# OSU-NLP-Group/saev

Hardware: AMD Instinct MI355X
Metric: activations/sec (train step), d_in=1024 x32 k=32 (higher is better)
Workload: dtype f32 (encoder: fp16 MFMA first pass with a rigorous error margin, survivors recomputed exactly in fp32; all else fp32)

## Files before the change

### saev_amd/csrc/ctx.h

```cpp
#pragma once
#include <hip/hip_runtime.h>

#include <algorithm>
#include <cmath>
#include <cstdio>
#include <cstdlib>
#include <cstring>
#include <string>
#include <vector>

#include "kernels.h"

constexpr int AUX_KSPLIT_MAX = 16;
constexpr int CAND_CAP = 4096;
constexpr int CAND_STRIDE = CAND_CAP + 256;
constexpr int TIMING_RING = 512;
constexpr int DEAD_LAG = 4;
constexpr int DEAD_RING = 16;
enum { AUX_NONE = 0, AUX_SMALL_DEVICE = 1, AUX_SMALL_HOST = 2, AUX_DENSE = 3 };

struct saev_ctx {
    saev_cfg cfg{};
    saev_debug_cfg dbg{};
    int device = 0;
// ... 42 lines not shown
    float2* row_proj = nullptr;
    float* enc_sq = nullptr;
    bool row_proj_valid = false, tail_proj_in_adam = false;
    bool wenc_t_pending = false;
    int64_t* toks = nullptr;
    int32_t *fired = nullptr, *dead = nullptr;
    int32_t* flags = nullptr;
    int32_t *chunk_starts = nullptr, *part_starts = nullptr, *work_latent = nullptr;
    float *dW_encT = nullptr, *partials = nullptr, *db_partials = nullptr;
    bool dws_ok = false;
    int dws_rows = 0;
    bool dws_pairs = false;
    float *gS = nullptr, *xS = nullptr, *dvp = nullptr;
    float* xS_ov = nullptr;
    float* xS_bwd = nullptr;
    float* dval_rows = nullptr;
    bool dval_fwd = false;
    float* wn2 = nullptr;
    float* sq_wave = nullptr;
    int sq_wave_n = 0;
    bool wn2_fresh = false;
    bool dval_pairs_ready = false;
    bool fused_forward = false;
    bool fwd_slices = false;
    bool fwd_step = false;
    float* rs_part = nullptr;
    float* xS_c = nullptr;
    int2 *pv = nullptr, *pv2 = nullptr;
    int32_t *plat = nullptr, *cut_lat = nullptr, *cut_list = nullptr;
    int32_t* lat_unused = nullptr;
    bool fused_step = false;
    bool unused_valid = false;
    int P = 1;
    int32_t cuts[MAX_PREFIXES] = {0};
    float* G = nullptr;
    float* GS = nullptr;
    int P_cap = 0;
    int n_dead_host = 0, k_use_host = 0;
    int64_t tokens_seen = 0;
    bool tracker_dirty = false;
    int nd_cap = 0;
    DeadRecord* rec_host = nullptr;
    DeadRecord* rec_dev = nullptr;
    hipEvent_t dead_ev[DEAD_RING];
    bool dead_ev_created = false;
    int64_t dead_steps = 0;
// ... 196 lines not shown
```

### saev_amd/csrc/ctx_backward.hip

```cpp
#include "ctx.h"

extern "C" {


int saev_backward_begin(saev_ctx* c, void* stream) {
    if (!c) return SAEV_INVALID_ARG;
    REQUIRE(c, !c->relu_train, SAEV_UNSUPPORTED, "saev_backward_begin: a ReLU training context runs its dense backward in one piece (saev_step_backward)");
    REQUIRE(c, c->x_last && c->training_last, SAEV_INVALID_ARG, "saev_backward_begin: no training forward in flight");
    REQUIRE(c, c->grads, SAEV_NOT_BOUND, "gradient buffer not bound");
    hipStream_t s = (hipStream_t)stream;
    const int S = c->cfg.d_sae, D = c->cfg.d_model, K = c->cfg.top_k;
    const bool ov = c->ov_x != nullptr;
    const int n = ov ? c->ov_n : c->n_last;
    const int words = ((n + 31) / 32 + 7) / 8 * 8;
    c->row_proj_valid = false;
    CscArgs a{};
    a.idx = ov ? c->ov_idx : c->idx; a.code_stride = K; a.k = K; a.k_dev = nullptr; a.n_rows = n; a.S = S;
    a.bitmap = c->bitmap; a.words = words; a.grp_prefix = c->grp_prefix; a.scan_totals = c->scan_totals;
    a.counts = c->counts; a.starts = c->starts; a.pairs = c->pairs;
    a.chunk_starts = c->chunk_starts; a.part_starts = c->part_starts; a.work_latent = c->work_latent;
    const bool ov_slices = ov && c->dws_ok && c->P_last == 1 && n <= c->back_rows;
    c->dws_pairs = ov ? ov_slices : c->dws_rows == n;
    if (ov_slices) {
        c->xS_bwd = c->xS;
        if (!c->followers.empty()) {
            if (c->xS_ov == nullptr) {
                int rca = alloc(c, &c->xS_ov, (size_t)c->back_rows * D);
                if (rca != SAEV_OK) return rca;
            }
            c->xS_bwd = c->xS_ov;
        }
        HIPCHK(c, launch_slice_major_copy(c->ov_g, c->ov_x, n, D, c->gS, c->xS_bwd, s));
        c->dws_rows = 0;
    }
    c->csc_epoch = c->csc_epoch == 0x7fffffff ? 1 : c->csc_epoch + 1;
    a.epoch = c->dbg.csc_route == 2 ? 0 : c->csc_epoch;
    if (c->dws_pairs) {
        a.zero_word = c->cut_list;
        a.pv = c->pv; a.plat = c->plat; a.val = ov ? c->ov_val : c->val;
        a.P = c->P_last;
        for (int p = 0; p < c->P_last; ++p) a.cuts[p] = c->cuts_last[p];
        if (!ov && c->dval_fwd) { a.pv2 = c->pv2; a.dval = c->dval_rows; }
    }
    c->dval_pairs_ready = c->dws_pairs && a.pv2 != nullptr;
    if (c->fused_step && c->dws_pairs) { a.pairs = nullptr; a.chunk_starts = nullptr; a.part_starts = nullptr; a.work_latent = nullptr; }
    const float* gmat = ov ? c->ov_g : (c->P_last > 1 ? c->G : c->g);
    const bool prefilled = !ov && c->bitmap_prefill_words == words && c->bitmap_prefill_rows == n;
    HIPCHK(c, launch_csc_build(a, s, c->bitmap_clean && words <= c->bitmap_clean_words, gmat, D, (long)c->P_last * D,
                               c->colsum_partials, c->grads + c->off_b_dec, prefilled));
    c->bitmap_prefill_words = 0;
    c->last_backward_gathered = ov;
    c->bitmap_clean = false;
    c->bitmap_words_last = words;
    if (c->aux_route != AUX_NONE) {
        int rc = auxk_backward(c, s);
        if (rc != SAEV_OK) return rc;
    }
    return SAEV_OK;
}

int saev_backward_rows(saev_ctx* c, int32_t lat_lo, int32_t lat_hi, void* stream) {
    return saev_backward_rows_part(c, lat_lo, lat_hi, 0, stream);
}

int saev_backward_rows_part(saev_ctx* c, int32_t lat_lo, int32_t lat_hi, int32_t part, void* stream) {
    if (!c) return SAEV_INVALID_ARG;
    REQUIRE(c, !c->relu_train, SAEV_UNSUPPORTED, "saev_backward_rows: a ReLU training context runs its dense backward in one piece, over all latents (saev_step_backward)");
    REQUIRE(c, part >= 0 && part <= 2, SAEV_INVALID_ARG, "saev_backward_rows_part: part must be 0 (both), 1 (decoder) or 2 (encoder)");
    REQUIRE(c, c->x_last && c->training_last && c->grads, SAEV_INVALID_ARG, "saev_backward_rows: call saev_backward_begin first");
    const int S = c->cfg.d_sae, D = c->cfg.d_model, K = c->cfg.top_k;
    const bool ov = c->ov_x != nullptr;
    const int n = ov ? c->ov_n : c->n_last;
    REQUIRE(c, 0 <= lat_lo && lat_lo < lat_hi && lat_hi <= S, SAEV_INVALID_ARG, "saev_backward_rows: bad latent range");
    REQUIRE(c, !c->btk || (part == 0 && lat_lo == 0 && lat_hi == S), SAEV_UNSUPPORTED,
            "saev_backward_rows: a BatchTopK context runs the backward over all latents in one part");
    hipStream_t s = (hipStream_t)stream;
    DwRowsArgs a{};
    a.starts = c->starts; a.chunk_starts = c->chunk_starts; a.work_latent = c->work_latent;
    a.part_starts = c->part_starts; a.pairs = c->pairs; a.val = ov ? c->ov_val : c->val; a.W_dec = c->params + c->off_W_dec;
    a.g = ov ? c->ov_g : (c->P_last > 1 ? c->G : c->g);
    a.x = ov ? c->ov_x : c->x_last;
    a.D = D; a.S = S; a.k_dev = nullptr; a.accumulate = 0;
    a.P = c->P_last;
    for (int p = 0; p < c->P_last; ++p) a.cuts[p] = c->cuts_last[p];
    a.dW_dec = c->grads + c->off_W_dec; a.dW_encT = c->dW_encT; a.db_enc = c->grads + c->off_b_enc;
    a.partials = c->partials; a.db_partials = c->db_partials;
    a.lat_lo = lat_lo; a.lat_hi = lat_hi;
    a.part = part; a.dval = c->dval_pairs;
    const bool all_rows = part == 0 && lat_lo == 0 && lat_hi == S;
    const bool clears = part != 2 && lat_lo == 0 && lat_hi == S && c->bitmap_words_last > 0;
    if (clears) { a.clear_bitmap = c->bitmap; a.clear_words = c->bitmap_words_last; }
    a.row_proj = all_rows ? c->row_proj : nullptr; a.project = c->cfg.remove_parallel_grads ? 1 : 0;
    a.enc_sq = all_rows ? c->enc_sq : nullptr;
    const int max_work = (lat_hi - lat_lo) + (int)(((long)n * K + DW_CHUNK - 1) / DW_CHUNK);
    if (lat_lo == 0 && lat_hi == S && c->dws_pairs && (ov || c->dws_rows == n)) {
        DwSlicesArgs w{};
        w.starts = c->starts; w.pv = c->pv; w.pv2 = c->pv2; w.plat = c->plat; w.gS = c->P_last > 1 ? c->GS : c->gS; w.W_dec = a.W_dec; w.P = c->P_last;
        w.xS = ov ? c->xS_bwd : (c->fwd_step ? c->xS_c : c->xS);
        w.n_rows = n; w.D = D; w.S = S; w.pair_cap = (int)((long)c->back_rows * K);
        w.dvp = c->dvp; w.dW_dec = a.dW_dec; w.dW_encT = a.dW_encT; w.db_enc = a.db_enc;
        const size_t runs_cap = ((size_t)w.pair_cap + DWS_RUN - 1) / DWS_RUN;
        w.part_dec = c->partials; w.part_enc = c->partials + 2 * runs_cap * D;
        w.cut_lat = c->cut_lat; w.cut_list = c->cut_list;
        w.lat_unused = (all_rows && c->fused_step) ? c->lat_unused : nullptr;
        c->unused_valid = w.lat_unused != nullptr;
        w.row_proj = a.row_proj; w.project = a.project; w.enc_sq = a.enc_sq;
        w.clear_bitmap = a.clear_bitmap; w.clear_words = a.clear_words;
        w.have_dval = c->dval_pairs_ready ? 1 : 0;
        c->sq_wave_n = 0;
        if (c->dval_pairs_ready && c->wn2_fresh && part == 0) {
            w.wn2 = c->wn2;
            if (c->fused_step && all_rows && c->sq_wave != nullptr && c->dbg.fin_route != 2) {
                c->sq_wave_n = dw_slices_waves(D, (int)((long)n * K));
                w.sq_wave_dec = c->sq_wave; w.sq_wave_enc = c->sq_wave + c->sq_wave_n;
            }
        }
        HIPCHK(c, launch_dw_slices(w, (int)((long)n * K), part, s));
    } else {
// ... 13 lines not shown
    if (ov && c->aux_route != AUX_NONE && part != 2 && lat_lo == 0)
        HIPCHK(c, launch_colsum(c->db_aux, 1, D, c->colsum_partials, c->grads + c->off_b_dec, 1, nullptr, s));
    c->row_proj_valid = all_rows;
    if (clears) { c->bitmap_clean = true; c->bitmap_clean_words = c->bitmap_words_last; }
    return SAEV_OK;
}

float* saev_grad_w_enc_t(saev_ctx* c) { return c ? c->dW_encT : nullptr; }

int saev_bind_w_enc_t(saev_ctx* c, float* scratch) {
    if (!c || !scratch) return SAEV_INVALID_ARG;
    c->dW_encT = scratch;
    return SAEV_OK;
}

int saev_copy_step_state(saev_ctx* c, int32_t n_rows, float* g_out, int32_t* idx_out, float* val_out, void* stream) {
    if (!c) return SAEV_INVALID_ARG;
    REQUIRE(c, !c->btk, SAEV_UNSUPPORTED, "saev_copy_step_state: not for a BatchTopK context (no sparse-state exchange)");
    REQUIRE(c, !c->relu_train, SAEV_UNSUPPORTED, "saev_copy_step_state: not for a ReLU training context (its step state is dense: no sparse-state exchange)");
    REQUIRE(c, c->n_last > 0 && c->training_last && n_rows == c->n_last, SAEV_INVALID_ARG,
            "saev_copy_step_state: n_rows must be the row count of the training forward in flight");
    hipStream_t s = (hipStream_t)stream;
    const size_t nk = (size_t)n_rows * c->cfg.top_k, nd = (size_t)n_rows * c->cfg.d_model * (size_t)c->P_last;
    if (g_out) HIPCHK(c, hipMemcpyAsync(g_out, c->P_last > 1 ? c->G : c->g, nd * sizeof(float), hipMemcpyDeviceToDevice, s));
    if (idx_out) HIPCHK(c, hipMemcpyAsync(idx_out, c->idx, nk * sizeof(int32_t), hipMemcpyDeviceToDevice, s));
    if (val_out) HIPCHK(c, hipMemcpyAsync(val_out, c->val, nk * sizeof(float), hipMemcpyDeviceToDevice, s));
    return SAEV_OK;
}

int saev_backward_override(saev_ctx* c, const float* x_all, const float* g_all, const int32_t* idx_all, const float* val_all,
                           int32_t n_all) {
    if (!c) return SAEV_INVALID_ARG;
    if (x_all == nullptr) { c->ov_x = nullptr; c->ov_n = 0; return SAEV_OK; }
    REQUIRE(c, !c->btk, SAEV_UNSUPPORTED, "saev_backward_override: not for a BatchTopK context (a batch-wide top-k over ranks needs a distributed select)");
    REQUIRE(c, !c->relu_train, SAEV_UNSUPPORTED, "saev_backward_override: not for a ReLU training context (one GPU: the dense backward runs over its own rows)");
    REQUIRE(c, g_all && idx_all && val_all && n_all > 0, SAEV_INVALID_ARG, "saev_backward_override: NULL buffer");
    REQUIRE(c, n_all <= c->back_rows, SAEV_INVALID_ARG,
            "saev_backward_override: the gathered row count exceeds saev_cfg.max_backward_rows (set it to the GLOBAL batch)");
    REQUIRE(c, c->x_last && c->training_last, SAEV_INVALID_ARG, "saev_backward_override: no training forward in flight");
    REQUIRE(c, ((uintptr_t)x_all % 16) == 0 && ((uintptr_t)g_all % 16) == 0, SAEV_INVALID_ARG, "x_all / g_all must be 16-byte aligned");
    c->ov_x = x_all; c->ov_g = g_all; c->ov_idx = idx_all; c->ov_val = val_all; c->ov_n = n_all;
    return SAEV_OK;
}

int32_t saev_aux_compact_rows(const saev_ctx* c) {
    if (!c || c->aux_route == AUX_NONE) return 0;
// ... 53 lines not shown
```

### saev_amd/csrc/ctx_forward.hip

```cpp
#include "ctx.h"

extern "C" {


int saev_normalize_w_dec(saev_ctx* c, void* stream) {
    if (!c) return SAEV_INVALID_ARG;
    REQUIRE(c, c->params, SAEV_NOT_BOUND, "parameters not bound");
    if (!c->cfg.normalize_w_dec) return SAEV_OK;
    HIPCHK(c, launch_normalize_rows(c->params + c->off_W_dec, c->cfg.d_sae, c->cfg.d_model, (hipStream_t)stream));
    return SAEV_OK;
}

static bool bind_x_sources(saev_ctx* c, const float* x, int n, bool allow_borrow) {
    saev_ctx* l = c->leader;
    const bool borrow = allow_borrow && l != nullptr && l->xprep_x == x && l->xprep_n == n && l->xprep_serial != c->leader_serial_seen;
    saev_ctx* src = borrow ? l : c;
    c->upper_c = src->upper; c->mu_c = src->mu; c->xnorm_c = src->xnorm; c->xabs_c = src->xabs_part; c->xs_c = src->xs;
    c->borrow_streamed = borrow && l->fwd_streamed && l->mu_keep != nullptr;
    if (c->borrow_streamed) c->mu_c = l->mu_keep;
    c->fwd_step = c->fwd_slices && (src == c || src->fwd_slices);
    c->xS_c = c->fwd_step ? src->xS : nullptr;
    if (borrow) c->leader_serial_seen = l->xprep_serial;
    return borrow;
}
// ... 230 lines not shown
            } else
            HIPCHK(c, launch_pre_encode(c->cand_cnt, n, c->gmax, ng * c->gmax_stride, f16r_mode ? c->xnorm_c : nullptr, c->cfg.d_model,
                                        c->wnorm_scratch, (S_ + 255) / 256, f16r_mode ? scl(c) : nullptr, const_cast<int32_t*>(pre_flag),
                                        c->wmax_prev, c->row_margin, c->flags + 1, s));
            timing_begin(c, s);
            int rc = run_encoder(c, x, n, EPI_TOPK, nullptr, pre_flag, 0, s);
            if (rc != SAEV_OK) return rc;
            timing_end(c, s);
            rc = select_stage(need_dense, 0, need_dense, nullptr, c->flags + 1, pre_flag);
            if (rc != SAEV_OK) return rc;
        }
    } else {
        HIPCHK(c, launch_init_i32(need_dense, 1, 1, s));
        HIPCHK(c, hipMemsetAsync(c->flags + 2, 0, 2 * sizeof(int32_t), s));
        timing_begin(c, s);
        timing_end(c, s);
    }
    int rc = run_encoder(c, x, n, EPI_DENSE, c->h_dense, need_dense, 1, s);
    if (rc != SAEV_OK) return rc;
    SelectDenseArgs sd{};
    sd.h = c->h_dense; sd.n_rows = n; sd.S = c->cfg.d_sae; sd.k = K;
    sd.idx_out = idx_out; sd.val_out = val_out; sd.out_stride = K;
    sd.enable_flag = need_dense; sd.enable_when = 1;
    HIPCHK(c, launch_select_dense(sd, s));
    return SAEV_OK;
}

int saev_encode_topk(saev_ctx* c, const float* x, int32_t n, int32_t* idx_out, float* val_out, void* stream) {
    if (!c) return SAEV_INVALID_ARG;
    REQUIRE(c, c->cfg.activation == SAEV_ACT_TOPK, SAEV_UNSUPPORTED,
            "saev_encode_topk: a TopK context only (ReLU: saev_encode_relu, BatchTopK: saev_encode_batch_topk)");
    REQUIRE(c, c->params, SAEV_NOT_BOUND, "parameters not bound");
    REQUIRE(c, x && idx_out && val_out && n > 0 && n <= c->cfg.max_batch, SAEV_INVALID_ARG,
            "saev_encode_topk: bad arguments (n_rows must be in 1..max_batch)");
    hipStream_t s = (hipStream_t)stream;
    HIPCHK(c, hipMemsetAsync(c->flags, 0, sizeof(int32_t), s));
    bind_x_sources(c, x, n, false);
    c->xprep_x = nullptr;
    c->stream_step = false;
    c->follow_stream = false;
    return encode_topk_impl(c, x, n, idx_out, val_out, c->flags, s);
}

int saev_scatter_dense(saev_ctx* c, const int32_t* idx, const float* val, int32_t n, int32_t k, float* f_out,
                       void* stream) {
    if (!c) return SAEV_INVALID_ARG;
// ... 246 lines not shown
        c->prep_valid = true;
    }
    if (wdec_ev != nullptr) HIPCHK(c, hipStreamWaitEvent(s, wdec_ev, 0));
    if (training) {
        c->wn2_fresh = false;
        if (c->cfg.normalize_w_dec) {
            HIPCHK(c, launch_normalize_rows(c->params + c->off_W_dec, S, D, s, c->wn2));
            c->wn2_fresh = c->wn2 != nullptr;
        }
    }

    DecodeArgs a{};
    a.x = x; a.idx = c->idx; a.val = c->val; a.code_stride = K; a.k = K;
    a.W_dec = c->params + c->off_W_dec; a.b_dec = c->params + c->off_b_dec;
    a.n_rows = n; a.D = D; a.S = S; a.idx_limit = S;
    a.upper = c->upper_c;
    a.gscale = 2.0f / ((float)n * (float)D * (float)c->P);
    a.training = training ? 1 : 0;
    a.g = c->g; a.x_hat = c->x_hat; a.fired = c->fired; a.rowstats = c->rowstats;
    c->dws_rows = 0;
    c->dval_fwd = false;
    if (training && c->dws_ok && (c->P == 1 || c->GS != nullptr)) { a.gS = c->P == 1 ? c->gS : c->GS; a.xS = c->fwd_step ? nullptr : c->xS; c->dws_rows = n; }
    if (c->dws_rows == n && c->dval_rows != nullptr && (c->P == 1 || decode_matry_forms_dval(D, K))) { a.dval_out = c->dval_rows; c->dval_fwd = true; }
    c->bitmap_prefill_words = 0;
    if (training && c->dbg.csc_route == 0 && c->bitmap != nullptr && c->bitmap_clean && !c->last_backward_gathered) {
        const int words = ((n + 31) / 32 + 7) / 8 * 8;
        if (words <= c->bitmap_clean_words) {
            a.csc_bitmap = c->bitmap; a.csc_words = words;
            c->bitmap_prefill_words = words; c->bitmap_prefill_rows = n;
            c->bitmap_clean = false;
        }
    }
    if (c->P > 1) {
        MatryArgs m{};
        m.P = c->P;
        for (int p = 0; p < c->P; ++p) m.cuts[p] = c->cuts[p];
        m.G = c->G;
        m.g_rows_all = c->fused_forward ? 0 : 1;
        HIPCHK(c, launch_decode_matry(a, m, s));
    } else {
        HIPCHK(c, launch_decode(a, s));
    }
    c->P_last = c->P;
    for (int p = 0; p < c->P; ++p) c->cuts_last[p] = c->cuts[p];
    const bool lists = !btk && fused_supported(c->cfg) && !(c->cfg.bound_mode != 0 && c->cfg.encoder_mode != SAEV_ENCODER_F32 && f16_ngroups(c) == 32);
    c->stats_pending = false;
// ... 12 lines not shown
```

### saev_amd/csrc/kernels.h

```cpp
#pragma once
#include <hip/hip_runtime.h>
#include <stdint.h>

#include <string>

#include "../../include/saev_amd.h"

enum { EPI_DENSE = 0, EPI_TOPK = 1 };

struct EncodeArgs {
    const float* x;
    const float* W_enc;
    const float* b_enc;
    int n_rows, D, S;
    int s_splits;
    float* h_out;
    int ngroups;
    int32_t* gmax;
    int gmax_stride;
    int32_t* cand_cnt;
    float* cand_val;
    int32_t* cand_idx;
    int cand_cap;
    int cand_stride;
    const int32_t* enable_flag;
    int enable_when;
};

size_t encode_gemm_smem_bytes();
hipError_t launch_encode_gemm(const EncodeArgs& a, int epi, hipStream_t stream);
int encode_gemm_tile_rows();
int encode_gemm_tile_latents();

struct SelectDenseArgs {
    const float* h;
    int n_rows, S;
    int k;
    const int32_t* k_dev;
    const int32_t* mask;
    int32_t* idx_out;
    float* val_out;
    int out_stride;
    const int32_t* enable_flag;
    int enable_when;
};
hipError_t launch_select_dense(const SelectDenseArgs& a, hipStream_t stream);

struct SelectCandArgs {
    const int32_t* cand_cnt;
    const float* cand_val;
    const int32_t* cand_idx;
    int cand_cap, cand_stride, n_rows, k;
    int32_t* idx_out;
    float* val_out;
    int out_stride;
    const int32_t* enable_flag;
    int enable_when;
    const float* row_margin;
    const float* x;
    const float* W_encT;
    const float* b_enc;
    int D;
    int32_t* surv_idx;
    float* surv_val;
    int32_t* surv_cnt;
    int32_t* refine_overflow;
    const int32_t* tau_max;
// ... 93 lines not shown
    int n_rows, S;
    uint32_t* bitmap;
    int words;
    int32_t* grp_prefix;
    int32_t* counts;
    int32_t* scan_totals;
    int32_t* starts;
    int2* pairs;
    int32_t* chunk_starts;
    int32_t* part_starts;
    int32_t* work_latent;
    int2* pv;
    int32_t* plat;
    const float* val;
    int2* pv2;
    const float* dval;
    int P;
    int32_t cuts[16];
    int32_t* zero_word;
    int32_t epoch;
};
hipError_t launch_csc_build(const CscArgs& a, hipStream_t stream, bool bitmap_clean = false, const float* colsum_m = nullptr,
                            int colsum_D = 0, long colsum_row_stride = 0, float* colsum_partials = nullptr,
                            float* colsum_out = nullptr, bool prefilled = false);

constexpr int DW_CHUNK = 64;

struct DwRowsArgs {
    const int32_t* starts;
    const int32_t* chunk_starts;
    const int32_t* work_latent;
    const int32_t* part_starts;
    const int2* pairs;
    const float* val;
    const float* W_dec;
    const float* g;
    const float* x;
    int D, S;
    int P;
    int32_t cuts[MAX_PREFIXES];
    const int32_t* k_dev;
    int accumulate;
    float* dW_dec;
    float* dW_encT;
    float* db_enc;
    float* partials;
    float* db_partials;
// ... 446 lines not shown
```

### saev_amd/csrc/select.hip

```cpp
#include "common.h"
#include "kernels.h"

namespace {

constexpr int SD_THREADS = 256;

__device__ __forceinline__ int block_excl_scan_256(int v, int* lds_wave_tot, int& total) {
    const int lane = threadIdx.x & 63, w = threadIdx.x >> 6;
    int incl = v;
#pragma unroll
    for (int o = 1; o < 64; o <<= 1) {
        int n = __shfl_up(incl, o, 64);
        if (lane >= o) incl += n;
    }
    if (lane == 63) lds_wave_tot[w] = incl;
    __syncthreads();
    int base = 0, tot = 0;
#pragma unroll
    for (int i = 0; i < 4; ++i) {
        const int t = lds_wave_tot[i];
        if (i < w) base += t;
        tot += t;
    }
    total = tot;
    __syncthreads();
    return base + incl - v;
}

__global__ __launch_bounds__(SD_THREADS) void select_dense_kernel(SelectDenseArgs a) {
    if (a.enable_flag != nullptr && (*a.enable_flag != 0) != (a.enable_when != 0)) return;
    __shared__ int hist[256];
    __shared__ int sh_digit, sh_need;
    __shared__ int wave_tot[4];

    const int row = blockIdx.x;
    const int S = a.S;
    int k = a.k_dev ? min(*a.k_dev, a.k) : a.k;
    if (a.k_dev && k <= 0) return;
    const float* h = a.h + (size_t)row * S;
    const int tid = threadIdx.x;
    const int S4 = S >> 2;

    uint32_t prefix = 0, pmask = 0;
    int need = k;

    for (int pass = 0; pass < 4; ++pass) {
        const int shift = 24 - 8 * pass;
        hist[tid] = 0;
        __syncthreads();
        for (int q = tid; q < S4; q += SD_THREADS) {
            const f32x4 v = *reinterpret_cast<const f32x4*>(h + 4 * q);
            int4 mk = {1, 1, 1, 1};
            if (a.mask) mk = *reinterpret_cast<const int4*>(a.mask + 4 * q);
            const int m[4] = {mk.x, mk.y, mk.z, mk.w};
#pragma unroll
            for (int e = 0; e < 4; ++e) {
                const uint32_t key = f2ukey(v[e]);
                if (m[e] != 0 && (key & pmask) == prefix) atomicAdd(&hist[(key >> shift) & 255], 1);
            }
        }
        __syncthreads();
        if (tid < 64) {
            const int c0 = hist[4 * tid], c1 = hist[4 * tid + 1], c2 = hist[4 * tid + 2], c3 = hist[4 * tid + 3];
            const int c = c0 + c1 + c2 + c3;
// ... 47 lines not shown
        const int neq = feq[0] + feq[1] + feq[2] + feq[3];
        int tot;
        const int ex = block_excl_scan_256(ngt | (neq << 16), wave_tot, tot);
        int gt_before = base_gt + (ex & 0xFFFF);
        int eq_before = base_eq + (ex >> 16);
#pragma unroll
        for (int e = 0; e < 4; ++e) {
            if (flg[e]) {
                const int pos = gt_before + min(eq_before, need);
                oi[pos] = 4 * q + e;
                ov[pos] = v[e];
                ++gt_before;
            } else if (feq[e]) {
                if (eq_before < need) {
                    const int pos = gt_before + eq_before;
                    oi[pos] = 4 * q + e;
                    ov[pos] = v[e];
                }
                ++eq_before;
            }
        }
        base_gt += tot & 0xFFFF;
        base_eq += tot >> 16;
    }
}


__device__ __forceinline__ float wave_reduce_scatter8(float (&p)[8], int lane) {
    int bit = 32;
#pragma unroll
    for (int h = 4; h >= 1; h >>= 1, bit >>= 1) {
        const bool up = (lane & bit) != 0;
#pragma unroll
        for (int i = 0; i < h; ++i) {
            const float keep = up ? p[i + h] : p[i];
            const float send = up ? p[i] : p[i + h];
            p[i] = keep + __shfl_xor(send, bit, 64);
        }
    }
    float r = p[0];
    for (; bit >= 1; bit >>= 1) r += __shfl_xor(r, bit, 64);
    return r;
}

__device__ __forceinline__ void sort_by_idx_and_store(const SelectCandArgs& a, int row, int k, int32_t my_idx, float my_val,
                                                      int lane) {
// ... 724 lines not shown
    if (state[5] > 0.f) { state[5] -= 1.f; g = 1; }
    *gate = g;
}
__global__ void heur_update_kernel(float* state, const int32_t* bad, const float* cand_mean, int k, const int32_t* gate) {
    if (threadIdx.x != 0 || *gate != 0) return;
    float z = state[0];
    state[2] += 1.f;
    if (*bad != 0) {
        z -= 0.3f;
        state[1] += 1.f;
        state[4] += 1.f;
        if (state[4] >= 3.f) { state[4] = 0.f; state[5] = 256.f; z = 1.5f; }
    } else {
        state[4] = 0.f;
        if (*cand_mean > 3.f * (float)k) z += 0.002f;
    }
    state[0] = fminf(fmaxf(z, 0.5f), 3.5f);
}

}

hipError_t launch_select_dense(const SelectDenseArgs& a, hipStream_t stream) {
    if (a.n_rows <= 0) return hipSuccess;
    hipLaunchKernelGGL(select_dense_kernel, dim3(a.n_rows), dim3(SD_THREADS), 0, stream, a);
    return hipGetLastError();
}

hipError_t launch_select_cand(const SelectCandArgs& a, hipStream_t stream) {
    if (a.n_rows <= 0) return hipSuccess;
    if (a.cand_cap > 4096 || (a.sum_part != nullptr && a.cand_cap > REFINE_CAP)) return hipErrorInvalidValue;
    if (a.k > 32) hipLaunchKernelGGL(select_cand_kernel<true>, dim3((a.n_rows + 3) / 4), dim3(256), 0, stream, a);
    else hipLaunchKernelGGL(select_cand_kernel<false>, dim3((a.n_rows + 3) / 4), dim3(256), 0, stream, a);
    return hipGetLastError();
}

hipError_t launch_init_i32(int32_t* p, int32_t v, int n, hipStream_t stream) {
    if (n <= 0) return hipSuccess;
    hipLaunchKernelGGL(init_i32_kernel, dim3((n + 255) / 256), dim3(256), 0, stream, p, v, n);
    return hipGetLastError();
}

hipError_t launch_encoder_init(int32_t* cand_cnt, int n_rows, int32_t* gmax, int n_gmax, hipStream_t stream, int32_t* tau_max,
                               const int32_t* enable_flag, int enable_when) {
    const int n = n_rows > n_gmax ? n_rows : n_gmax;
    if (n <= 0) return hipSuccess;
    hipLaunchKernelGGL(encoder_init_kernel, dim3((n + 255) / 256), dim3(256), 0, stream, cand_cnt, n_rows, gmax, n_gmax, tau_max,
                       enable_flag, enable_when);
// ... 96 lines not shown
```

### saev_amd/csrc/sparse.hip

```cpp
#include "common.h"
#include "kernels.h"

namespace {

template <int NV>
__device__ __forceinline__ void gather_rows_accum(f32x4 (&acc)[NV], const float* __restrict__ W, int D, int D4,
                                                  const int32_t* idx_row, const float* val_row, int k, int limit,
                                                  int lane) {
    for (int j0 = 0; j0 < k; j0 += 64) {
        const int cnt = min(64, k - j0);
        int32_t my_i = -1;
        float my_v = 0.f;
        if (lane < cnt) { my_i = idx_row[j0 + lane]; my_v = val_row[j0 + lane]; }
#pragma unroll 4
        for (int jj = 0; jj < cnt; ++jj) {
            const int32_t i = __shfl(my_i, jj, 64);
            const float v = __shfl(my_v, jj, 64);
            if (i < 0 || i >= limit) continue;
            const f32x4* wr = reinterpret_cast<const f32x4*>(W + (size_t)i * D);
#pragma unroll
            for (int n = 0; n < NV; ++n) {
                const int q = lane + 64 * n;
                if (q < D4) {
                    const f32x4 w = wr[q];
// ... 69 lines not shown
        return;
    }
    const float u = a.upper ? fmaxf(*a.upper, 1e-12f) : 1.0f;
    float sse_scaled = 0.f;
    double sse64 = 0.0, sumsq64 = 0.0;
    f32x4 g[NV];
    const f32x4* xr = reinterpret_cast<const f32x4*>(a.x + (size_t)row * D);
#pragma unroll
    for (int n = 0; n < NV; ++n) {
        const int q = lane + 64 * n;
        g[n] = f32x4{0.f, 0.f, 0.f, 0.f};
        if (q < D4) {
            const f32x4 xv = xr[q];
            if (a.x_hat) reinterpret_cast<f32x4*>(a.x_hat + (size_t)row * D)[q] = acc[n];
#pragma unroll
            for (int e = 0; e < 4; ++e) {
                const float t = acc[n][e] / u - xv[e] / u;
                sse_scaled += t * t * u * u;
                g[n][e] = a.gscale * t * u;
                const float r = xv[e] - acc[n][e];
                sse64 += (double)r * (double)r;
                sumsq64 += (double)xv[e] * (double)xv[e];
            }
            if (a.training) reinterpret_cast<f32x4*>(a.g + (size_t)row * D)[q] = g[n];
            if (a.training && a.gS != nullptr) {
                const size_t o = ((size_t)(q >> 3) * a.n_rows + row) * 8 + (q & 7);
                reinterpret_cast<f32x4*>(a.gS)[o] = g[n];
                if (a.xS != nullptr) reinterpret_cast<f32x4*>(a.xS)[o] = xv;
            }
        }
    }
    float l0 = 0.f, l1 = 0.f;
    for (int j = lane; j < a.k; j += 64) {
        const int32_t i = idx_row[j];
        const float v = val_row[j];
        if (i >= 0 && v != 0.f) {
            l0 += 1.f;
            l1 += fabsf(v);
            if (a.training && a.fired) a.fired[i] = 1;
        }
        csc_mark(a, i, row);
    }
    if (a.rowstats) {
        sse_scaled = wave_sum(sse_scaled);
        l0 = wave_sum(l0);
        l1 = wave_sum(l1);
        sse64 = wave_sum_d(sse64);
// ... 42 lines not shown
#pragma unroll
        for (int j = 0; j < 32; ++j) {
            const int i = __builtin_amdgcn_readlane(my_i, 32 * h + j);
            const float v = __builtin_bit_cast(float, __builtin_amdgcn_readlane(__builtin_bit_cast(int, raw_v), 32 * h + j));
            if (i >= 0) acc += v * wv[j];
        }
        __builtin_amdgcn_sched_barrier(0);
    }
    if (a.x_hat) reinterpret_cast<f32x4*>(a.x_hat + (size_t)row * a.D)[q] = acc;
    const float u = a.upper ? fmaxf(*a.upper, 1e-12f) : 1.0f;
    float sse_scaled = 0.f;
    double sse64 = 0.0, sumsq64 = 0.0;
    f32x4 g;
#pragma unroll
    for (int e = 0; e < 4; ++e) {
        const float t = acc[e] / u - xv[e] / u;
        sse_scaled += t * t * u * u;
        g[e] = a.gscale * t * u;
        const float r = xv[e] - acc[e];
        sse64 += (double)r * (double)r;
        sumsq64 += (double)xv[e] * (double)xv[e];
    }
    if (a.training) {
        reinterpret_cast<f32x4*>(a.g + (size_t)row * a.D)[q] = g;
        if (a.gS != nullptr) {
            const size_t o = ((size_t)(q >> 3) * a.n_rows + row) * 8 + (q & 7);
            reinterpret_cast<f32x4*>(a.gS)[o] = g;
            if (a.xS != nullptr) reinterpret_cast<f32x4*>(a.xS)[o] = xv;
        }
    }
#pragma unroll
    for (int hh = 0; hh < KH; ++hh) {
        const int h = KH - 1 - hh;
        if (hh > 0) {
#pragma unroll
            for (int j = 0; j < 32; ++j) {
                const int i = __builtin_amdgcn_readlane(my_i, 32 * h + j);
                const i32x4_ t = __builtin_amdgcn_raw_buffer_load_b128(wres, voff, (uint32_t)max(i, 0) * (uint32_t)(D4 * 16), 0);
                wv[j] = f32x4{__int_as_float(t[0]), __int_as_float(t[1]), __int_as_float(t[2]), __int_as_float(t[3])};
            }
            __builtin_amdgcn_sched_barrier(0);
        }
        float pd[32];
#pragma unroll
        for (int j = 0; j < 32; ++j) pd[j] = (g[0] * wv[j][0] + g[1] * wv[j][1]) + (g[2] * wv[j][2] + g[3] * wv[j][3]);
        const float r = wave_reduce_scatter32(pd, lane);
        if ((lane & 1) == 0) sh_dv[w][32 * h + (lane >> 1)] = r;
// ... 1220 lines not shown
    if (k_dev && col_mult > 0 && (int)blockIdx.x * 64 >= *k_dev * col_mult) return;
    __shared__ float part[4][64];
    const int col = threadIdx.x & 63, slice = threadIdx.x >> 6;
    const int d = blockIdx.x * 64 + col;
    float s0 = 0.f, s1 = 0.f, s2 = 0.f, s3 = 0.f;
    if (d < D) {
        int b = slice;
        for (; b + 12 < n_blocks; b += 16) {
            s0 += partials[(size_t)b * D + d];
            s1 += partials[(size_t)(b + 4) * D + d];
            s2 += partials[(size_t)(b + 8) * D + d];
            s3 += partials[(size_t)(b + 12) * D + d];
        }
        for (; b < n_blocks; b += 4) s0 += partials[(size_t)b * D + d];
    }
    part[slice][col] = (s0 + s1) + (s2 + s3);
    __syncthreads();
    if (slice == 0 && d < D) {
        const float s = (part[0][col] + part[1][col]) + (part[2][col] + part[3][col]);
        out[d] = accumulate ? out[d] + s * out_scale : s * out_scale;
    }
}

struct ColsumPlain { const float* m; int n_rows, D; float* partials; long row_stride; float* out; int n_blocks; };
__device__ __forceinline__ void colsum_partial_plain(const ColsumPlain& c, int bid) {
    const int r0 = bid * 64, r1 = min(c.n_rows, r0 + 64);
    for (int q = threadIdx.x; q < (c.D >> 2); q += 256) {
        f32x4 s = {0.f, 0.f, 0.f, 0.f};
        int r = r0;
        for (; r + 8 <= r1; r += 8) {
            f32x4 v[8];
#pragma unroll
            for (int u = 0; u < 8; ++u) v[u] = reinterpret_cast<const f32x4*>(c.m + (size_t)(r + u) * c.row_stride)[q];
            s += ((v[0] + v[1]) + (v[2] + v[3])) + ((v[4] + v[5]) + (v[6] + v[7]));
        }
        for (; r < r1; ++r) s += reinterpret_cast<const f32x4*>(c.m + (size_t)r * c.row_stride)[q];
        reinterpret_cast<f32x4*>(c.partials + (size_t)bid * c.D)[q] = s;
    }
}
__device__ __forceinline__ void colsum_final_plain(const ColsumPlain& c, int bid, float (&part)[4][64]) {
    const int col = threadIdx.x & 63, slice = threadIdx.x >> 6;
    const int d = bid * 64 + col;
    float s0 = 0.f, s1 = 0.f, s2 = 0.f, s3 = 0.f;
    if (d < c.D && slice < 4) {
        int b = slice;
        for (; b + 12 < c.n_blocks; b += 16) {
            s0 += c.partials[(size_t)b * c.D + d];
            s1 += c.partials[(size_t)(b + 4) * c.D + d];
            s2 += c.partials[(size_t)(b + 8) * c.D + d];
            s3 += c.partials[(size_t)(b + 12) * c.D + d];
        }
        for (; b < c.n_blocks; b += 4) s0 += c.partials[(size_t)b * c.D + d];
    }
    if (slice < 4) part[slice][col] = (s0 + s1) + (s2 + s3);
    __syncthreads();
    if (slice == 0 && d < c.D) c.out[d] = ((part[0][col] + part[1][col]) + (part[2][col] + part[3][col])) * 1.0f;
}
__global__ __launch_bounds__(1024) void csc_scan_fused_kernel(CscArgs a, int n_scan, ColsumPlain c, int have_colsum) {
    __shared__ int wave_tot[16][3];
// ... 119 lines not shown
        static bool attr_set = false;
        if (!attr_set) {
            const void* fns[4] = {reinterpret_cast<const void*>(&decode_matry_q_kernel<1>), reinterpret_cast<const void*>(&decode_matry_q_kernel<2>),
                                  reinterpret_cast<const void*>(&decode_matry_q_kernel<3>), reinterpret_cast<const void*>(&decode_matry_q_kernel<4>)};
            for (const void* f : fns) {
                hipError_t e = hipFuncSetAttribute(f, hipFuncAttributeMaxDynamicSharedMemorySize, MAX_PREFIXES * 1024 * (int)sizeof(float));
                if (e != hipSuccess) return e;
            }
            attr_set = true;
        }
        switch (a.D / 256) {
            case 1: hipLaunchKernelGGL(decode_matry_q_kernel<1>, dim3(a.n_rows), dim3(64), smem, stream, a, m); break;
            case 2: hipLaunchKernelGGL(decode_matry_q_kernel<2>, dim3(a.n_rows), dim3(128), smem, stream, a, m); break;
            case 3: hipLaunchKernelGGL(decode_matry_q_kernel<3>, dim3(a.n_rows), dim3(192), smem, stream, a, m); break;
            default: hipLaunchKernelGGL(decode_matry_q_kernel<4>, dim3(a.n_rows), dim3(256), smem, stream, a, m); break;
        }
        return hipGetLastError();
    }
    return dispatch_nv(a.D, [&](auto nv) {
        hipLaunchKernelGGL(decode_matry_kernel<decltype(nv)::value>, dim3((a.n_rows + 3) / 4), dim3(256), 0, stream, a, m);
    });
}
hipError_t launch_csc_build(const CscArgs& a, hipStream_t stream, bool bitmap_clean, const float* colsum_m, int colsum_D,
                            long colsum_row_stride, float* colsum_partials, float* colsum_out, bool prefilled) {
    if (a.n_rows <= 0) return hipSuccess;
    const long n = (long)a.n_rows * a.k;
    const int blocks = prefilled ? 0 : (int)std::min<long>((n + 255) / 256, 4096);
    const int place_blocks = (int)std::min<long>((std::max<long>(n, a.S) + 255) / 256, 8192);
    if (!bitmap_clean && !prefilled) hipLaunchKernelGGL(csc_clear_kernel, dim3(2048), dim3(256), 0, stream, a);
    const int n_scan = (a.S + 1023) / 1024;
    ColsumPlain c{colsum_m, a.n_rows, colsum_D, colsum_partials, colsum_row_stride > 0 ? colsum_row_stride : (long)colsum_D,
                  colsum_out, (a.n_rows + 63) / 64};
    int colsum_in_scan = 0;
    if (colsum_m != nullptr && prefilled && a.epoch != 0) {
        hipLaunchKernelGGL(csc_count_colpart_kernel, dim3((a.S + 3) / 4 + c.n_blocks), dim3(256), 0, stream, a, (a.S + 3) / 4, c);
        colsum_in_scan = 1;
    } else if (colsum_m != nullptr) {
        hipLaunchKernelGGL(csc_fill_colsum_kernel, dim3(blocks + c.n_blocks), dim3(256), 0, stream, a, blocks, c);
        hipLaunchKernelGGL(csc_count_colsum_kernel, dim3((a.S + 3) / 4 + (colsum_D + 63) / 64), dim3(256), 0, stream, a, (a.S + 3) / 4, c);
    } else {
        if (blocks > 0) hipLaunchKernelGGL(csc_fill_kernel, dim3(blocks), dim3(256), 0, stream, a);
        hipLaunchKernelGGL(csc_count_kernel, dim3((a.S + 3) / 4), dim3(256), 0, stream, a);
    }
    if (a.epoch != 0 && n_scan <= 128) {
        hipLaunchKernelGGL(csc_scan_fused_kernel, dim3(n_scan + (colsum_in_scan ? (colsum_D + 63) / 64 : 0)), dim3(1024), 0, stream, a, n_scan, c,
                           colsum_in_scan);
    } else {
        hipLaunchKernelGGL(csc_scan_block_kernel, dim3(n_scan), dim3(1024), 0, stream, a);
        hipLaunchKernelGGL(csc_scan_offset_kernel, dim3(n_scan), dim3(1024), 0, stream, a);
    }
    hipLaunchKernelGGL(csc_place_kernel, dim3(place_blocks), dim3(256), 0, stream, a);
    return hipGetLastError();
}
hipError_t launch_dw_rows(const DwRowsArgs& a, int max_work, hipStream_t stream) {
    return dispatch_nv(a.D, [&](auto nv) {
// ... 70 lines not shown
```

### saev_amd/csrc/split.hip

```cpp
#include "common.h"
#include "kernels.h"

namespace {

typedef _Float16 half8 __attribute__((ext_vector_type(8)));

typedef __bf16 bf16x8 __attribute__((ext_vector_type(8)));

__device__ __forceinline__ half8 split8(const float (&v)[8], int part) {
    half8 o;
#pragma unroll
    for (int e = 0; e < 8; ++e) {
        const _Float16 h = (_Float16)v[e];
        o[e] = part == 0 ? h : (_Float16)(v[e] - (float)h);
    }
    return o;
}

__device__ __forceinline__ half8 round8_bf16(const float (&v)[8]) {
    bf16x8 o;
#pragma unroll
    for (int e = 0; e < 8; ++e) o[e] = (__bf16)v[e];
    return __builtin_bit_cast(half8, o);
}
// ... 261 lines not shown
        h ^= h >> 15; h *= 2246822519u; h ^= h >> 13;
        const uint32_t d = h % (uint32_t)a.D, sidx = (h >> 8) % (uint32_t)a.S;
        const float w = a.W_enc[(size_t)d * a.S + sidx], c = a.WeS[((size_t)(d >> 5) * a.S + sidx) * 32 + (d & 31)];
        if (__float_as_uint(w) != __float_as_uint(c)) atomicOr(a.stale, 1);
    }
    if (a.stale != nullptr && i >= 128 && i < 192) {
        bool differs = false;
        for (int sidx = bid * 64 + (i - 128); sidx < a.S; sidx += (int)gridDim.x * 64)
            differs |= __float_as_uint(a.b_enc[sidx]) != __float_as_uint(a.b_seen[sidx]);
        if (differs) atomicOr(a.stale, 1);
    }
}

__global__ __launch_bounds__(256) void bias_finish_kernel(const double* __restrict__ dot_part,
                                                          const float* __restrict__ sq_part, int nks, int S, int S_pad,
                                                          const float* __restrict__ w_scale, const float* __restrict__ b_enc,
                                                          float* __restrict__ b_shift, float* __restrict__ wg_max,
                                                          float* __restrict__ b_seen) {
    __shared__ float sh[3][4];
    const int sidx = blockIdx.x * 256 + threadIdx.x;
    float out = 0.f, nrm = 0.f, dnrm = 0.f;
    if (sidx < S) {
        double acc = 0.0, sq = 0.0, dsq = 0.0;
        for (int ks = 0; ks < nks; ++ks) {
            acc += dot_part[(size_t)ks * S_pad + sidx];
            sq += (double)sq_part[(size_t)ks * S_pad + sidx];
            dsq += (double)sq_part[(size_t)(nks + ks) * S_pad + sidx];
        }
        const double sc = (double)(*w_scale);
        const float be = b_enc[sidx];
        out = (float)(acc / sc + (double)be);
        b_shift[sidx] = out;
        if (b_seen != nullptr) b_seen[sidx] = be;
        nrm = (float)(sqrt(sq) / sc) * 1.000001f;
        dnrm = (float)(sqrt(dsq) / sc) * 1.00001f;
    }
    float m = fabsf(out);
    for (int o = 32; o > 0; o >>= 1) { m = fmaxf(m, __shfl_xor(m, o, 64)); nrm = fmaxf(nrm, __shfl_xor(nrm, o, 64)); dnrm = fmaxf(dnrm, __shfl_xor(dnrm, o, 64)); }
    if ((threadIdx.x & 63) == 0) { sh[0][threadIdx.x >> 6] = m; sh[1][threadIdx.x >> 6] = nrm; sh[2][threadIdx.x >> 6] = dnrm; }
    __syncthreads();
    if (threadIdx.x < 3) {
        const float* q = sh[threadIdx.x];
        wg_max[threadIdx.x * gridDim.x + blockIdx.x] = fmaxf(fmaxf(q[0], q[1]), fmaxf(q[2], q[3]));
    }
}


}

hipError_t launch_split_rows(const float* x, int n, int D, int Dp, void* xs, int mode, hipStream_t stream, float scale,
// ... 58 lines not shown
```

Before: 6.264 million.

## Drop row-major gradient in fused step, grid-stride dense select, batch bias-finish loads

When the fused training step runs with a single prefix and slice-major gradient rows, the forward stops writing the row-major gradient matrix. The decoder-bias column sum then reads the slice-major copy through a new stride mode, which removes one full n×D write per step. Separately, the dense top-k select kernel becomes grid-stride with a capped grid of 1024 blocks for fused configs, and the bias-finish reduction batches 16 partial loads before accumulating so more loads are in flight. Latent-range backward calls and copy_step_state now fail with an error when the row-major gradient was skipped.

Result: faster. 6.332 million (median of 6 runs) (+1.1%).

```diff
diff --git a/saev_amd/csrc/ctx.h b/saev_amd/csrc/ctx.h
--- a/saev_amd/csrc/ctx.h
+++ b/saev_amd/csrc/ctx.h
@@ -88,6 +88,7 @@
     bool wn2_fresh = false;
     bool dval_pairs_ready = false;
     bool fused_forward = false;
+    bool g_rows_valid = true;
     bool fwd_slices = false;
     bool fwd_step = false;
     float* rs_part = nullptr;
diff --git a/saev_amd/csrc/ctx_backward.hip b/saev_amd/csrc/ctx_backward.hip
--- a/saev_amd/csrc/ctx_backward.hip
+++ b/saev_amd/csrc/ctx_backward.hip
@@ -45,9 +45,14 @@
     c->dval_pairs_ready = c->dws_pairs && a.pv2 != nullptr;
     if (c->fused_step && c->dws_pairs) { a.pairs = nullptr; a.chunk_starts = nullptr; a.part_starts = nullptr; a.work_latent = nullptr; }
     const float* gmat = ov ? c->ov_g : (c->P_last > 1 ? c->G : c->g);
+    const bool g_slices = !ov && c->P_last == 1 && !c->g_rows_valid;
+    if (g_slices) {
+        REQUIRE(c, c->dws_rows == n, SAEV_INVALID_ARG, "saev_backward_begin: the forward in flight left no gradient rows");
+        gmat = c->gS;
+    }
     const bool prefilled = !ov && c->bitmap_prefill_words == words && c->bitmap_prefill_rows == n;
     HIPCHK(c, launch_csc_build(a, s, c->bitmap_clean && words <= c->bitmap_clean_words, gmat, D, (long)c->P_last * D,
-                               c->colsum_partials, c->grads + c->off_b_dec, prefilled));
+                               c->colsum_partials, c->grads + c->off_b_dec, prefilled, g_slices));
     c->bitmap_prefill_words = 0;
     c->last_backward_gathered = ov;
     c->bitmap_clean = false;
@@ -79,6 +84,9 @@
     a.starts = c->starts; a.chunk_starts = c->chunk_starts; a.work_latent = c->work_latent;
     a.part_starts = c->part_starts; a.pairs = c->pairs; a.val = ov ? c->ov_val : c->val; a.W_dec = c->params + c->off_W_dec;
     a.g = ov ? c->ov_g : (c->P_last > 1 ? c->G : c->g);
+    const bool slices_all = lat_lo == 0 && lat_hi == S && c->dws_pairs && (ov || c->dws_rows == n);
+    REQUIRE(c, ov || c->P_last > 1 || c->g_rows_valid || slices_all, SAEV_INVALID_ARG,
+            "saev_backward_rows: the fused step's forward keeps no row-major gradient (a latent range needs the phase forward)");
     a.x = ov ? c->ov_x : c->x_last;
     a.D = D; a.S = S; a.k_dev = nullptr; a.accumulate = 0;
     a.P = c->P_last;
@@ -93,7 +101,7 @@
     a.row_proj = all_rows ? c->row_proj : nullptr; a.project = c->cfg.remove_parallel_grads ? 1 : 0;
     a.enc_sq = all_rows ? c->enc_sq : nullptr;
     const int max_work = (lat_hi - lat_lo) + (int)(((long)n * K + DW_CHUNK - 1) / DW_CHUNK);
-    if (lat_lo == 0 && lat_hi == S && c->dws_pairs && (ov || c->dws_rows == n)) {
+    if (slices_all) {
         DwSlicesArgs w{};
         w.starts = c->starts; w.pv = c->pv; w.pv2 = c->pv2; w.plat = c->plat; w.gS = c->P_last > 1 ? c->GS : c->gS; w.W_dec = a.W_dec; w.P = c->P_last;
         w.xS = ov ? c->xS_bwd : (c->fwd_step ? c->xS_c : c->xS);
@@ -153,6 +161,8 @@
             "saev_copy_step_state: n_rows must be the row count of the training forward in flight");
     hipStream_t s = (hipStream_t)stream;
     const size_t nk = (size_t)n_rows * c->cfg.top_k, nd = (size_t)n_rows * c->cfg.d_model * (size_t)c->P_last;
+    REQUIRE(c, !g_out || c->P_last > 1 || c->g_rows_valid, SAEV_INVALID_ARG,
+            "saev_copy_step_state: the fused step's forward keeps no row-major gradient (use saev_step_forward)");
     if (g_out) HIPCHK(c, hipMemcpyAsync(g_out, c->P_last > 1 ? c->G : c->g, nd * sizeof(float), hipMemcpyDeviceToDevice, s));
     if (idx_out) HIPCHK(c, hipMemcpyAsync(idx_out, c->idx, nk * sizeof(int32_t), hipMemcpyDeviceToDevice, s));
     if (val_out) HIPCHK(c, hipMemcpyAsync(val_out, c->val, nk * sizeof(float), hipMemcpyDeviceToDevice, s));
diff --git a/saev_amd/csrc/ctx_forward.hip b/saev_amd/csrc/ctx_forward.hip
--- a/saev_amd/csrc/ctx_forward.hip
+++ b/saev_amd/csrc/ctx_forward.hip
@@ -276,6 +276,7 @@
     sd.h = c->h_dense; sd.n_rows = n; sd.S = c->cfg.d_sae; sd.k = K;
     sd.idx_out = idx_out; sd.val_out = val_out; sd.out_stride = K;
     sd.enable_flag = need_dense; sd.enable_when = 1;
+    if (fused_supported(c->cfg)) sd.walk_grid = 4 * 256;
     HIPCHK(c, launch_select_dense(sd, s));
     return SAEV_OK;
 }
@@ -568,6 +569,8 @@
     c->dval_fwd = false;
     if (training && c->dws_ok && (c->P == 1 || c->GS != nullptr)) { a.gS = c->P == 1 ? c->gS : c->GS; a.xS = c->fwd_step ? nullptr : c->xS; c->dws_rows = n; }
     if (c->dws_rows == n && c->dval_rows != nullptr && (c->P == 1 || decode_matry_forms_dval(D, K))) { a.dval_out = c->dval_rows; c->dval_fwd = true; }
+    c->g_rows_valid = !(c->train_fused && training && c->P == 1 && c->dws_rows == n);
+    if (!c->g_rows_valid) a.g = nullptr;
     c->bitmap_prefill_words = 0;
     if (training && c->dbg.csc_route == 0 && c->bitmap != nullptr && c->bitmap_clean && !c->last_backward_gathered) {
         const int words = ((n + 31) / 32 + 7) / 8 * 8;
diff --git a/saev_amd/csrc/kernels.h b/saev_amd/csrc/kernels.h
--- a/saev_amd/csrc/kernels.h
+++ b/saev_amd/csrc/kernels.h
@@ -43,6 +43,7 @@
     int out_stride;
     const int32_t* enable_flag;
     int enable_when;
+    int walk_grid;
 };
 hipError_t launch_select_dense(const SelectDenseArgs& a, hipStream_t stream);
 
@@ -182,7 +183,8 @@
 };
 hipError_t launch_csc_build(const CscArgs& a, hipStream_t stream, bool bitmap_clean = false, const float* colsum_m = nullptr,
                             int colsum_D = 0, long colsum_row_stride = 0, float* colsum_partials = nullptr,
-                            float* colsum_out = nullptr, bool prefilled = false);
+                            float* colsum_out = nullptr, bool prefilled = false,
+                            bool colsum_slice_major = false);
 
 constexpr int DW_CHUNK = 64;
 
diff --git a/saev_amd/csrc/select.hip b/saev_amd/csrc/select.hip
--- a/saev_amd/csrc/select.hip
+++ b/saev_amd/csrc/select.hip
@@ -33,13 +33,13 @@
     __shared__ int sh_digit, sh_need;
     __shared__ int wave_tot[4];
 
-    const int row = blockIdx.x;
     const int S = a.S;
     int k = a.k_dev ? min(*a.k_dev, a.k) : a.k;
     if (a.k_dev && k <= 0) return;
-    const float* h = a.h + (size_t)row * S;
     const int tid = threadIdx.x;
     const int S4 = S >> 2;
+    for (int row = blockIdx.x; row < a.n_rows; row += gridDim.x) {
+    const float* h = a.h + (size_t)row * S;
 
     uint32_t prefix = 0, pmask = 0;
     int need = k;
@@ -133,6 +133,8 @@
         }
         base_gt += tot & 0xFFFF;
         base_eq += tot >> 16;
+    }
+    __syncthreads();
     }
 }
 
@@ -903,7 +905,8 @@
 
 hipError_t launch_select_dense(const SelectDenseArgs& a, hipStream_t stream) {
     if (a.n_rows <= 0) return hipSuccess;
-    hipLaunchKernelGGL(select_dense_kernel, dim3(a.n_rows), dim3(SD_THREADS), 0, stream, a);
+    const int grid = (a.walk_grid > 0 && a.walk_grid < a.n_rows) ? a.walk_grid : a.n_rows;
+    hipLaunchKernelGGL(select_dense_kernel, dim3(grid), dim3(SD_THREADS), 0, stream, a);
     return hipGetLastError();
 }
 
diff --git a/saev_amd/csrc/sparse.hip b/saev_amd/csrc/sparse.hip
--- a/saev_amd/csrc/sparse.hip
+++ b/saev_amd/csrc/sparse.hip
@@ -115,7 +115,7 @@
                 sse64 += (double)r * (double)r;
                 sumsq64 += (double)xv[e] * (double)xv[e];
             }
-            if (a.training) reinterpret_cast<f32x4*>(a.g + (size_t)row * D)[q] = g[n];
+            if (a.training && a.g != nullptr) reinterpret_cast<f32x4*>(a.g + (size_t)row * D)[q] = g[n];
             if (a.training && a.gS != nullptr) {
                 const size_t o = ((size_t)(q >> 3) * a.n_rows + row) * 8 + (q & 7);
                 reinterpret_cast<f32x4*>(a.gS)[o] = g[n];
@@ -204,7 +204,7 @@
         sumsq64 += (double)xv[e] * (double)xv[e];
     }
     if (a.training) {
-        reinterpret_cast<f32x4*>(a.g + (size_t)row * a.D)[q] = g;
+        if (a.g != nullptr) reinterpret_cast<f32x4*>(a.g + (size_t)row * a.D)[q] = g;
         if (a.gS != nullptr) {
             const size_t o = ((size_t)(q >> 3) * a.n_rows + row) * 8 + (q & 7);
             reinterpret_cast<f32x4*>(a.gS)[o] = g;
@@ -1471,19 +1471,22 @@
     }
 }
 
-struct ColsumPlain { const float* m; int n_rows, D; float* partials; long row_stride; float* out; int n_blocks; };
+struct ColsumPlain { const float* m; int n_rows, D; float* partials; long row_stride; float* out; int n_blocks; int slice_major; };
 __device__ __forceinline__ void colsum_partial_plain(const ColsumPlain& c, int bid) {
     const int r0 = bid * 64, r1 = min(c.n_rows, r0 + 64);
     for (int q = threadIdx.x; q < (c.D >> 2); q += 256) {
+        const f32x4* const base = c.slice_major ? reinterpret_cast<const f32x4*>(c.m) + (size_t)(q >> 3) * c.n_rows * 8 + (q & 7)
+                                                : reinterpret_cast<const f32x4*>(c.m) + q;
+        const size_t pitch = c.slice_major ? (size_t)8 : (size_t)(c.row_stride >> 2);
         f32x4 s = {0.f, 0.f, 0.f, 0.f};
         int r = r0;
         for (; r + 8 <= r1; r += 8) {
             f32x4 v[8];
 #pragma unroll
-            for (int u = 0; u < 8; ++u) v[u] = reinterpret_cast<const f32x4*>(c.m + (size_t)(r + u) * c.row_stride)[q];
+            for (int u = 0; u < 8; ++u) v[u] = base[(size_t)(r + u) * pitch];
             s += ((v[0] + v[1]) + (v[2] + v[3])) + ((v[4] + v[5]) + (v[6] + v[7]));
         }
-        for (; r < r1; ++r) s += reinterpret_cast<const f32x4*>(c.m + (size_t)r * c.row_stride)[q];
+        for (; r < r1; ++r) s += base[(size_t)r * pitch];
         reinterpret_cast<f32x4*>(c.partials + (size_t)bid * c.D)[q] = s;
     }
 }
@@ -1649,7 +1652,7 @@
     });
 }
 hipError_t launch_csc_build(const CscArgs& a, hipStream_t stream, bool bitmap_clean, const float* colsum_m, int colsum_D,
-                            long colsum_row_stride, float* colsum_partials, float* colsum_out, bool prefilled) {
+                            long colsum_row_stride, float* colsum_partials, float* colsum_out, bool prefilled, bool colsum_slice_major) {
     if (a.n_rows <= 0) return hipSuccess;
     const long n = (long)a.n_rows * a.k;
     const int blocks = prefilled ? 0 : (int)std::min<long>((n + 255) / 256, 4096);
@@ -1657,7 +1660,7 @@
     if (!bitmap_clean && !prefilled) hipLaunchKernelGGL(csc_clear_kernel, dim3(2048), dim3(256), 0, stream, a);
     const int n_scan = (a.S + 1023) / 1024;
     ColsumPlain c{colsum_m, a.n_rows, colsum_D, colsum_partials, colsum_row_stride > 0 ? colsum_row_stride : (long)colsum_D,
-                  colsum_out, (a.n_rows + 63) / 64};
+                  colsum_out, (a.n_rows + 63) / 64, colsum_slice_major ? 1 : 0};
     int colsum_in_scan = 0;
     if (colsum_m != nullptr && prefilled && a.epoch != 0) {
         hipLaunchKernelGGL(csc_count_colpart_kernel, dim3((a.S + 3) / 4 + c.n_blocks), dim3(256), 0, stream, a, (a.S + 3) / 4, c);
diff --git a/saev_amd/csrc/split.hip b/saev_amd/csrc/split.hip
--- a/saev_amd/csrc/split.hip
+++ b/saev_amd/csrc/split.hip
@@ -307,10 +307,26 @@
     float out = 0.f, nrm = 0.f, dnrm = 0.f;
     if (sidx < S) {
         double acc = 0.0, sq = 0.0, dsq = 0.0;
-        for (int ks = 0; ks < nks; ++ks) {
-            acc += dot_part[(size_t)ks * S_pad + sidx];
-            sq += (double)sq_part[(size_t)ks * S_pad + sidx];
-            dsq += (double)sq_part[(size_t)(nks + ks) * S_pad + sidx];
+        constexpr int CH = 16;
+#pragma unroll 1
+        for (int k0 = 0; k0 < nks; k0 += CH) {
+            double va[CH];
+            float vs[CH], vd[CH];
+#pragma unroll
+            for (int j = 0; j < CH; ++j) {
+                const int ks = min(k0 + j, nks - 1);
+                va[j] = dot_part[(size_t)ks * S_pad + sidx];
+                vs[j] = sq_part[(size_t)ks * S_pad + sidx];
+                vd[j] = sq_part[(size_t)(nks + ks) * S_pad + sidx];
+            }
+            __builtin_amdgcn_sched_barrier(0);
+#pragma unroll
+            for (int j = 0; j < CH; ++j)
+                if (k0 + j < nks) {
+                    acc += va[j];
+                    sq += (double)vs[j];
+                    dsq += (double)vd[j];
+                }
         }
         const double sc = (double)(*w_scale);
         const float be = b_enc[sidx];
```
